# vincentjzy/OpenCorr

Measured on NVIDIA H100. Metric: POIs/sec (FFTCC+ICGN to convergence), higher is better.
Workload: dtype f32

## Files before the change

opencorr_b200/csrc/fft32.cuh:

```cuda
#pragma once
#include "ocb_common.cuh"

namespace ocb {

__host__ __device__ constexpr int brev5(int i) {
	return ((i & 1) << 4) | ((i & 2) << 2) | (i & 4) | ((i & 8) >> 2) | ((i & 16) >> 4);
}

__device__ __forceinline__ float tw32_cos(int k) {
	switch (k) {
	case 0: return 1.0f;
	case 1: return 0.98078528040323044913f;
	case 2: return 0.92387953251128675613f;
	case 3: return 0.83146961230254523708f;
	case 4: return 0.70710678118654752440f;
	case 5: return 0.55557023301960222474f;
	case 6: return 0.38268343236508977173f;
	case 7: return 0.19509032201612826785f;
	case 8: return 0.0f;
	case 9: return -0.19509032201612826785f;
	case 10: return -0.38268343236508977173f;
	case 11: return -0.55557023301960222474f;
	case 12: return -0.70710678118654752440f;
	case 13: return -0.83146961230254523708f;
	case 14: return -0.92387953251128675613f;
	default: return -0.98078528040323044913f;
	}
}
__device__ __forceinline__ float tw32_sin(int k) { return k < 8 ? tw32_cos(8 - k) : tw32_cos(k - 8); }

template <bool INV>
__device__ __forceinline__ void mul_tw32(float xr, float xi, int k, float& yr, float& yi) {
	if (k == 0) {
		yr = xr;
		yi = xi;
	} else if (k == 8) {
		yr = INV ? -xi : xi;
		yi = INV ? xr : -xr;
	} else {
		const float c = tw32_cos(k), s = INV ? -tw32_sin(k) : tw32_sin(k);
		yr = fmaf(xr, c, xi * s);
		yi = fmaf(xi, c, -xr * s);
	}
}

template <bool INV, int HALF>
__device__ __forceinline__ void fft32_dif_stage(float* re, float* im) {
#pragma unroll
	for (int base = 0; base < 32; base += 2 * HALF) {
#pragma unroll
		for (int k = 0; k < HALF; k++) {
			const int i = base + k, j = i + HALF;
			const float ar = re[i], ai = im[i], br = re[j], bi = im[j];
			re[i] = ar + br;
			im[i] = ai + bi;
			mul_tw32<INV>(ar - br, ai - bi, k * (16 / HALF), re[j], im[j]);
		}
	}
}

template <bool INV, int HALF>
__device__ __forceinline__ void fft32_dit_stage(float* re, float* im) {
#pragma unroll
	for (int base = 0; base < 32; base += 2 * HALF) {
#pragma unroll
		for (int k = 0; k < HALF; k++) {
			const int i = base + k, j = i + HALF;
			float tr, ti;
			mul_tw32<INV>(re[j], im[j], k * (16 / HALF), tr, ti);
			const float ar = re[i], ai = im[i];
			re[i] = ar + tr;
			im[i] = ai + ti;
			re[j] = ar - tr;
			im[j] = ai - ti;
		}
	}
}

template <bool INV>
__device__ __forceinline__ void fft32_dif(float* re, float* im) {
	fft32_dif_stage<INV, 16>(re, im);
	fft32_dif_stage<INV, 8>(re, im);
	fft32_dif_stage<INV, 4>(re, im);
	fft32_dif_stage<INV, 2>(re, im);
	fft32_dif_stage<INV, 1>(re, im);
}

template <bool INV>
__device__ __forceinline__ void fft32_dit(float* re, float* im) {
	fft32_dit_stage<INV, 1>(re, im);
	fft32_dit_stage<INV, 2>(re, im);
	fft32_dit_stage<INV, 4>(re, im);
	fft32_dit_stage<INV, 8>(re, im);
	fft32_dit_stage<INV, 16>(re, im);
}

}
```

opencorr_b200/csrc/fftcc2d_w32.cu:

```cuda
#include <stdlib.h>
#include <string.h>

#include "fft32.cuh"
#include "fftcc_common.cuh"
#include "ocb_kernels.h"
#include "ocb_tma.cuh"

namespace ocb {

constexpr int FFTW32_PITCH = 33;
constexpr int FFTW32_BOX_W = 36;
constexpr int FFTW32_TILE = 32 * FFTW32_BOX_W;

__global__ void __launch_bounds__(FFTW32_WARPS * 32) fftcc2d_w32_kernel(Image2D img, float* __restrict__ pois, int n_poi,
	const __grid_constant__ CUtensorMap tm_ref, const __grid_constant__ CUtensorMap tm_tar, int use_tma) {
	__shared__ __align__(128) float s_re[FFTW32_WARPS][FFTW32_TILE];
	__shared__ __align__(128) float s_im[FFTW32_WARPS][FFTW32_TILE];
	__shared__ __align__(8) uint64_t s_bar[FFTW32_WARPS];
	constexpr int R = 16, M = 32 * 32;
	const int lane = threadIdx.x & 31, warp = threadIdx.x >> 5;
	float* sre = s_re[warp];
	float* sim = s_im[warp];
	uint64_t* bar = &s_bar[warp];
	uint32_t bar_phase = 0;
	if (use_tma) {
		if (lane == 0) mbar_init(bar, 1);
		__syncwarp();
	}
	const int w = img.w, h = img.h;
	const int plane = (32 - lane) & 31;

	const int poi_stride = gridDim.x * FFTW32_WARPS;
	int poi = blockIdx.x * FFTW32_WARPS + warp;
	float rec_next = (poi < n_poi && lane < P2_N) ? pois[(size_t)poi * P2_N + lane] : 0.f;
	for (; poi < n_poi; poi += poi_stride) {
		float* P = pois + (size_t)poi * P2_N;
		const float rec = rec_next;
		if (poi + poi_stride < n_poi && lane < P2_N) rec_next = pois[(size_t)(poi + poi_stride) * P2_N + lane];
		const float px = __shfl_sync(0xffffffffu, rec, P2_X), py = __shfl_sync(0xffffffffu, rec, P2_Y);
		const float u0 = __shfl_sync(0xffffffffu, rec, P2_DEF + D2_U), v0 = __shfl_sync(0xffffffffu, rec, P2_DEF + D2_V);
		if (fftcc2d_skip(px, py, u0, v0, R, R, w, h)) continue;
		float re[32], im[32];
		{
			float sa = 0.f, sb = 0.f;
			if (use_tma && px == floorf(px) && py == floorf(py) && u0 == floorf(u0) && v0 == floorf(v0)) {
				const int x0r = (int)px - R, y0r = (int)py - R, x0t = (int)(px + u0) - R, y0t = (int)(py + v0) - R;
				const int axr = floor4(x0r), axt = floor4(x0t);
				if (lane == 0) {
					fence_proxy_async();
					mbar_expect_tx(bar, (uint32_t)(2 * FFTW32_TILE * sizeof(float)));
					tma_load_2d(sre, &tm_ref, axr, y0r, bar);
					tma_load_2d(sim, &tm_tar, axt, y0t, bar);
				}
				mbar_wait(bar, bar_phase);
				bar_phase ^= 1;
				const float* cr = sre + (x0r - axr) + lane;
				const float* ci = sim + (x0t - axt) + lane;
#pragma unroll
				for (int r = 0; r < 32; r++) {
					re[r] = cr[r * FFTW32_BOX_W];
					im[r] = ci[r * FFTW32_BOX_W];
					sa += re[r];
					sb += im[r];
				}
			} else {
				const float rpx = px + lane - R;
				const int ax = (int)rpx, bx = (int)(rpx + u0);
#pragma unroll
				for (int r = 0; r < 32; r++) {
					const float rpy = py + r - R;
					re[r] = __ldg(img.ref + (size_t)(int)rpy * w + ax);
					im[r] = __ldg(img.tar + (size_t)(int)(rpy + v0) * w + bx);
					sa += re[r];
					sb += im[r];
				}
			}
			sa = warp_sum(sa) / (float)M;
			sb = warp_sum(sb) / (float)M;
#pragma unroll
			for (int r = 0; r < 32; r++) {
				re[r] -= sa;
				im[r] -= sb;
			}
		}
		float na = 0.f, nb = 0.f;
#pragma unroll
		for (int r = 0; r < 32; r++) {
			na = fmaf(re[r], re[r], na);
			nb = fmaf(im[r], im[r], nb);
		}
		na = warp_sum(na);
		nb = warp_sum(nb);

		fft32_dif<false>(re, im);
		__syncwarp();
#pragma unroll
		for (int i = 0; i < 32; i++) {
			sre[brev5(i) * FFTW32_PITCH + lane] = re[i];
			sim[brev5(i) * FFTW32_PITCH + lane] = im[i];
		}
		__syncwarp();
#pragma unroll
		for (int i = 0; i < 32; i++) {
			re[i] = sre[lane * FFTW32_PITCH + i];
			im[i] = sim[lane * FFTW32_PITCH + i];
		}
		fft32_dif<false>(re, im);

#pragma unroll
		for (int i = 0; i < 32; i++) {
			const int ip = brev5((32 - brev5(i)) & 31);
			if (ip < i) continue;
			const float pr_i = __shfl_sync(0xffffffffu, re[i], plane), pi_i = __shfl_sync(0xffffffffu, im[i], plane);
			if (ip == i) {
				cross_spectrum(re[i], im[i], pr_i, pi_i);
			} else {
				const float pr_p = __shfl_sync(0xffffffffu, re[ip], plane), pi_p = __shfl_sync(0xffffffffu, im[ip], plane);
				cross_spectrum(re[i], im[i], pr_p, pi_p);
				cross_spectrum(re[ip], im[ip], pr_i, pi_i);
			}
		}

		fft32_dit<true>(re, im);
		__syncwarp();
#pragma unroll
		for (int i = 0; i < 32; i++) {
			sre[lane * FFTW32_PITCH + i] = re[i];
			sim[lane * FFTW32_PITCH + i] = im[i];
		}
		__syncwarp();
#pragma unroll
		for (int i = 0; i < 32; i++) {
			re[i] = sre[brev5(i) * FFTW32_PITCH + lane];
			im[i] = sim[brev5(i) * FFTW32_PITCH + lane];
		}
		fft32_dit<true>(re, im);

		float bv = -2.f;
		int bi = 0;
#pragma unroll
		for (int y = 0; y < 32; y++) {
			if (re[y] > bv) { bv = re[y]; bi = y * 32 + lane; }
		}
		warp_argmax(bv, bi);
		{
			const Fftcc2dResult res = fftcc2d_result(bv, bi, na, nb, R, R, u0, v0);
			float out = 0.f;
			if (lane == P2_DEF + D2_U) out = res.u;
			if (lane == P2_DEF + D2_V) out = res.v;
			if (lane == P2_U0) out = u0;
			if (lane == P2_V0) out = v0;
			if (lane == P2_ZNCC) out = res.zncc;
			if (lane == P2_DEF + D2_U || lane == P2_DEF + D2_V || lane == P2_U0 || lane == P2_V0 || lane == P2_ZNCC) P[lane] = out;
		}
		__syncwarp();
	}
}

int fftcc2d_w32_launch(const Image2D& img, float* d_pois, size_t n, int grid, cudaStream_t stream, cudaError_t* err) {
	CUtensorMap tm_ref, tm_tar;
	memset(&tm_ref, 0, sizeof(tm_ref));
	memset(&tm_tar, 0, sizeof(tm_tar));
	const int dims[2] = { img.w, img.h }, box[2] = { FFTW32_BOX_W, 32 };
	const int use_tma = !getenv("OCB_NO_TMA") && tma_make_map(&tm_ref, img.ref, 2, dims, box) && tma_make_map(&tm_tar, img.tar, 2, dims, box);
	fftcc2d_w32_kernel<<<grid, FFTW32_WARPS * 32, 0, stream>>>(img, d_pois, (int)n, tm_ref, tm_tar, use_tma);
	*err = cudaGetLastError();
	return *err == cudaSuccess ? 0 : -2;
}

}
```

opencorr_b200/csrc/fftcc_common.cuh:

```cuda
#pragma once
#include "ocb_common.cuh"

namespace ocb {

__device__ __forceinline__ bool fftcc2d_skip(float px, float py, float u0, float v0, int rx, int ry, int w, int h) {
	return (int)px < rx || (int)px >= w - rx || (int)py < ry || (int)py >= h - ry || (int)(px + u0) < rx || (int)(px + u0) >= w - rx
		|| (int)(py + v0) < ry || (int)(py + v0) >= h - ry || is_nan_f(px) || is_nan_f(py) || is_nan_f(u0) || is_nan_f(v0);
}

__device__ __forceinline__ bool fftcc3d_skip(float px, float py, float pz, float u0, float v0, float w0, int rx, int ry, int rz, int dx, int dy,
	int dz) {
	const int sx = 2 * rx, sy = 2 * ry, sz = 2 * rz;
	const int x0 = (int)(px - rx), y0 = (int)(py - ry), z0 = (int)(pz - rz);
	const int x1 = (int)(px + (sx - 1) - rx), y1 = (int)(py + (sy - 1) - ry), z1 = (int)(pz + (sz - 1) - rz);
	const int tx0 = (int)(px - rx + u0), ty0 = (int)(py - ry + v0), tz0 = (int)(pz - rz + w0);
	const int tx1 = (int)(px + (sx - 1) - rx + u0), ty1 = (int)(py + (sy - 1) - ry + v0), tz1 = (int)(pz + (sz - 1) - rz + w0);
	return x0 < 0 || y0 < 0 || z0 < 0 || x1 >= dx || y1 >= dy || z1 >= dz || tx0 < 0 || ty0 < 0 || tz0 < 0 || tx1 >= dx || ty1 >= dy || tz1 >= dz
		|| px - rx < 0 || py - ry < 0 || pz - rz < 0 || px - rx + u0 < 0 || py - ry + v0 < 0 || pz - rz + w0 < 0
		|| is_nan_f(px) || is_nan_f(py) || is_nan_f(pz) || is_nan_f(u0) || is_nan_f(v0) || is_nan_f(w0);
}

__device__ __forceinline__ void cross_spectrum(float& re, float& im, float nr, float ni) {
	const float Ar = 0.5f * (re + nr), Ai = 0.5f * (im - ni);
	const float dr = 0.5f * (re - nr), di = 0.5f * (im + ni);
	const float Br = di, Bi = -dr;
	re = Ar * Br + Ai * Bi;
	im = Ar * Bi - Ai * Br;
}

__device__ __forceinline__ void argmax_merge(float& bv, int& bi, float v, int i) {
	if (v > bv || (v == bv && i < bi)) { bv = v; bi = i; }
}
__device__ __forceinline__ void warp_argmax(float& bv, int& bi) {
#pragma unroll
	for (int o = 16; o > 0; o >>= 1) {
		const float ov = __shfl_xor_sync(0xffffffffu, bv, o);
		const int oi = __shfl_xor_sync(0xffffffffu, bi, o);
		argmax_merge(bv, bi, ov, oi);
	}
}

__device__ __forceinline__ void fftcc_constant_window(float& bv, int& bi, float na, float nb) {
	if (na == 0.f || nb == 0.f) { bv = 0.f; bi = 0; }
}
__device__ __forceinline__ float fftcc_zncc(float bv, float na, float nb, int m) { return bv / (sqrtf(na * nb) * (float)m); }
__device__ __forceinline__ int fftcc_wrap(int d, int r) { return d > r ? d - 2 * r : d; }

struct Fftcc2dResult {
	float u, v, zncc;
};
__device__ __forceinline__ Fftcc2dResult fftcc2d_result(float bv, int bi, float na, float nb, int rx, int ry, float u0, float v0) {
	fftcc_constant_window(bv, bi, na, nb);
	const int sw = 2 * rx;
	const unsigned k = (unsigned)bi;
	return { (float)fftcc_wrap((int)(k % sw), rx) + u0, (float)fftcc_wrap((int)(k / sw), ry) + v0, fftcc_zncc(bv, na, nb, sw * 2 * ry) };
}
__device__ __forceinline__ void fftcc2d_store(float* P, float bv, int bi, float na, float nb, int rx, int ry, float u0, float v0) {
	const Fftcc2dResult r = fftcc2d_result(bv, bi, na, nb, rx, ry, u0, v0);
	P[P2_DEF + D2_U] = r.u;
	P[P2_DEF + D2_V] = r.v;
	P[P2_U0] = u0;
	P[P2_V0] = v0;
	P[P2_ZNCC] = r.zncc;
}

__device__ __forceinline__ void fftcc3d_store(float* P, float bv, int bi, float na, float nb, int rx, int ry, int rz, float u0, float v0, float w0) {
	fftcc_constant_window(bv, bi, na, nb);
	const int sx = 2 * rx, sy = 2 * ry;
	const unsigned k = (unsigned)bi;
	P[P3_DEF + 0] = (float)fftcc_wrap((int)(k % sx), rx) + u0;
	P[P3_DEF + 4] = (float)fftcc_wrap((int)(k / sx % sy), ry) + v0;
	P[P3_DEF + 8] = (float)fftcc_wrap((int)(k / (sx * sy)), rz) + w0;
	P[P3_U0] = u0;
	P[P3_V0] = v0;
	P[P3_W0] = w0;
	P[P3_ZNCC] = fftcc_zncc(bv, na, nb, sx * sy * 2 * rz);
}

}
```

Measured before the change: 50.44 million.

## Exploit real-valued correlation output with half-size inverse FFT and float2 transposes

Replaces the full 32x32 complex inverse FFT with a real-output split: one 32-point pass becomes a twiddle pre-step plus a 16-point FFT. The second pass is handled by splitting lanes into two halves that each do a 16-point FFT over half the rows. The transpose buffers are merged into one float2 shared tile so each element moves with one vector access. The cross-spectrum drops its 0.5 scaling, and the factor is restored once at the argmax. This trims FFT arithmetic and shared-memory traffic, but the index mapping and argmax tie-breaking logic become more intricate.

```diff
diff --git a/opencorr_b200/csrc/fft32.cuh b/opencorr_b200/csrc/fft32.cuh
--- a/opencorr_b200/csrc/fft32.cuh
+++ b/opencorr_b200/csrc/fft32.cuh
@@ -44,10 +44,10 @@
 	}
 }
 
-template <bool INV, int HALF>
-__device__ __forceinline__ void fft32_dif_stage(float* re, float* im) {
+template <int N, bool INV, int HALF>
+__device__ __forceinline__ void fft_dif_stage(float* re, float* im) {
 #pragma unroll
-	for (int base = 0; base < 32; base += 2 * HALF) {
+	for (int base = 0; base < N; base += 2 * HALF) {
 #pragma unroll
 		for (int k = 0; k < HALF; k++) {
 			const int i = base + k, j = i + HALF;
@@ -59,10 +59,10 @@
 	}
 }
 
-template <bool INV, int HALF>
-__device__ __forceinline__ void fft32_dit_stage(float* re, float* im) {
+template <int N, bool INV, int HALF>
+__device__ __forceinline__ void fft_dit_stage(float* re, float* im) {
 #pragma unroll
-	for (int base = 0; base < 32; base += 2 * HALF) {
+	for (int base = 0; base < N; base += 2 * HALF) {
 #pragma unroll
 		for (int k = 0; k < HALF; k++) {
 			const int i = base + k, j = i + HALF;
@@ -79,20 +79,56 @@
 
 template <bool INV>
 __device__ __forceinline__ void fft32_dif(float* re, float* im) {
-	fft32_dif_stage<INV, 16>(re, im);
-	fft32_dif_stage<INV, 8>(re, im);
-	fft32_dif_stage<INV, 4>(re, im);
-	fft32_dif_stage<INV, 2>(re, im);
-	fft32_dif_stage<INV, 1>(re, im);
+	fft_dif_stage<32, INV, 16>(re, im);
+	fft_dif_stage<32, INV, 8>(re, im);
+	fft_dif_stage<32, INV, 4>(re, im);
+	fft_dif_stage<32, INV, 2>(re, im);
+	fft_dif_stage<32, INV, 1>(re, im);
 }
 
 template <bool INV>
 __device__ __forceinline__ void fft32_dit(float* re, float* im) {
-	fft32_dit_stage<INV, 1>(re, im);
-	fft32_dit_stage<INV, 2>(re, im);
-	fft32_dit_stage<INV, 4>(re, im);
-	fft32_dit_stage<INV, 8>(re, im);
-	fft32_dit_stage<INV, 16>(re, im);
+	fft_dit_stage<32, INV, 1>(re, im);
+	fft_dit_stage<32, INV, 2>(re, im);
+	fft_dit_stage<32, INV, 4>(re, im);
+	fft_dit_stage<32, INV, 8>(re, im);
+	fft_dit_stage<32, INV, 16>(re, im);
+}
+
+template <bool INV>
+__device__ __forceinline__ void fft16_dif(float* re, float* im) {
+	fft_dif_stage<16, INV, 8>(re, im);
+	fft_dif_stage<16, INV, 4>(re, im);
+	fft_dif_stage<16, INV, 2>(re, im);
+	fft_dif_stage<16, INV, 1>(re, im);
+}
+
+template <bool INV>
+__device__ __forceinline__ void fft16_dit(float* re, float* im) {
+	fft_dit_stage<16, INV, 1>(re, im);
+	fft_dit_stage<16, INV, 2>(re, im);
+	fft_dit_stage<16, INV, 4>(re, im);
+	fft_dit_stage<16, INV, 8>(re, im);
+}
+
+__device__ __forceinline__ void ifft32_real_split(float* re, float* im) {
+#pragma unroll
+	for (int j = 0; j < 16; j++) {
+		const int k = brev5(2 * j);
+		const float ar = re[2 * j], ai = im[2 * j], br = re[2 * j + 1], bi = im[2 * j + 1];
+		if (k == 0) {
+			re[j] = (ar + br) - (ai - bi);
+			im[j] = (ai + bi) + (ar - br);
+		} else if (k == 8) {
+			re[j] = br + br;
+			im[j] = bi + bi;
+		} else {
+			const float er = ar + br, ei = ai + bi, dr = ar - br, di = ai - bi;
+			const float c = tw32_cos(k), s = tw32_sin(k);
+			re[j] = fmaf(-dr, s, fmaf(-di, c, er));
+			im[j] = fmaf(dr, c, fmaf(-di, s, ei));
+		}
+	}
 }
 
 }
diff --git a/opencorr_b200/csrc/fftcc2d_w32.cu b/opencorr_b200/csrc/fftcc2d_w32.cu
--- a/opencorr_b200/csrc/fftcc2d_w32.cu
+++ b/opencorr_b200/csrc/fftcc2d_w32.cu
@@ -11,16 +11,17 @@
 constexpr int FFTW32_PITCH = 33;
 constexpr int FFTW32_BOX_W = 36;
 constexpr int FFTW32_TILE = 32 * FFTW32_BOX_W;
+static_assert(32 * FFTW32_PITCH * 2 <= 2 * FFTW32_TILE, "the transpose tile must fit in the two boxes");
 
 __global__ void __launch_bounds__(FFTW32_WARPS * 32) fftcc2d_w32_kernel(Image2D img, float* __restrict__ pois, int n_poi,
 	const __grid_constant__ CUtensorMap tm_ref, const __grid_constant__ CUtensorMap tm_tar, int use_tma) {
-	__shared__ __align__(128) float s_re[FFTW32_WARPS][FFTW32_TILE];
-	__shared__ __align__(128) float s_im[FFTW32_WARPS][FFTW32_TILE];
+	__shared__ __align__(128) float s_buf[FFTW32_WARPS][2 * FFTW32_TILE];
 	__shared__ __align__(8) uint64_t s_bar[FFTW32_WARPS];
 	constexpr int R = 16, M = 32 * 32;
 	const int lane = threadIdx.x & 31, warp = threadIdx.x >> 5;
-	float* sre = s_re[warp];
-	float* sim = s_im[warp];
+	float* sre = s_buf[warp];
+	float* sim = s_buf[warp] + FFTW32_TILE;
+	float2* st = reinterpret_cast<float2*>(s_buf[warp]);
 	uint64_t* bar = &s_bar[warp];
 	uint32_t bar_phase = 0;
 	if (use_tma) {
@@ -95,15 +96,13 @@
 		fft32_dif<false>(re, im);
 		__syncwarp();
 #pragma unroll
-		for (int i = 0; i < 32; i++) {
-			sre[brev5(i) * FFTW32_PITCH + lane] = re[i];
-			sim[brev5(i) * FFTW32_PITCH + lane] = im[i];
-		}
+		for (int i = 0; i < 32; i++) st[brev5(i) * FFTW32_PITCH + lane] = make_float2(re[i], im[i]);
 		__syncwarp();
 #pragma unroll
 		for (int i = 0; i < 32; i++) {
-			re[i] = sre[lane * FFTW32_PITCH + i];
-			im[i] = sim[lane * FFTW32_PITCH + i];
+			const float2 v = st[lane * FFTW32_PITCH + i];
+			re[i] = v.x;
+			im[i] = v.y;
 		}
 		fft32_dif<false>(re, im);
 
@@ -113,38 +112,50 @@
 			if (ip < i) continue;
 			const float pr_i = __shfl_sync(0xffffffffu, re[i], plane), pi_i = __shfl_sync(0xffffffffu, im[i], plane);
 			if (ip == i) {
-				cross_spectrum(re[i], im[i], pr_i, pi_i);
+				cross_spectrum4(re[i], im[i], pr_i, pi_i);
 			} else {
 				const float pr_p = __shfl_sync(0xffffffffu, re[ip], plane), pi_p = __shfl_sync(0xffffffffu, im[ip], plane);
-				cross_spectrum(re[i], im[i], pr_p, pi_p);
-				cross_spectrum(re[ip], im[ip], pr_i, pi_i);
+				cross_spectrum4(re[i], im[i], pr_p, pi_p);
+				cross_spectrum4(re[ip], im[ip], pr_i, pi_i);
 			}
 		}
 
-		fft32_dit<true>(re, im);
+		ifft32_real_split(re, im);
+		fft16_dit<true>(re, im);
 		__syncwarp();
 #pragma unroll
-		for (int i = 0; i < 32; i++) {
-			sre[lane * FFTW32_PITCH + i] = re[i];
-			sim[lane * FFTW32_PITCH + i] = im[i];
+		for (int n = 0; n < 16; n++) st[lane * FFTW32_PITCH + n] = make_float2(re[n], im[n]);
+		__syncwarp();
+		const int n = lane & 15, h = lane >> 4;
+		const float hf = (float)h, sgn = 1.f - 2.f * hf;
+#pragma unroll
+		for (int ky = 0; ky < 16; ky++) {
+			const float2 a = st[ky * FFTW32_PITCH + n], b = st[(ky + 16) * FFTW32_PITCH + n];
+			const float tr = fmaf(sgn, b.x, a.x), ti = fmaf(sgn, b.y, a.y);
+			if (ky == 0) {
+				re[ky] = tr;
+				im[ky] = ti;
+			} else {
+				const float cm1 = tw32_cos(ky) - 1.f, s = tw32_sin(ky);
+				re[ky] = fmaf(hf, fmaf(tr, cm1, -ti * s), tr);
+				im[ky] = fmaf(hf, fmaf(ti, cm1, tr * s), ti);
+			}
 		}
-		__syncwarp();
+		fft16_dif<true>(re, im);
+
+		float bv = -8.f;
+		const int i0 = h * 32 + 2 * n;
+		int bi = -i0;
 #pragma unroll
-		for (int i = 0; i < 32; i++) {
-			re[i] = sre[brev5(i) * FFTW32_PITCH + lane];
-			im[i] = sim[brev5(i) * FFTW32_PITCH + lane];
+		for (int m = 0; m < 16; m++) {
+			const int j = brev5(2 * m);
+			if (re[j] > bv) { bv = re[j]; bi = m * 64; }
+			if (im[j] > bv) { bv = im[j]; bi = m * 64 + 1; }
 		}
-		fft32_dit<true>(re, im);
-
-		float bv = -2.f;
-		int bi = 0;
-#pragma unroll
-		for (int y = 0; y < 32; y++) {
-			if (re[y] > bv) { bv = re[y]; bi = y * 32 + lane; }
-		}
+		bi += i0;
 		warp_argmax(bv, bi);
 		{
-			const Fftcc2dResult res = fftcc2d_result(bv, bi, na, nb, R, R, u0, v0);
+			const Fftcc2dResult res = fftcc2d_result(0.25f * bv, bi, na, nb, R, R, u0, v0);
 			float out = 0.f;
 			if (lane == P2_DEF + D2_U) out = res.u;
 			if (lane == P2_DEF + D2_V) out = res.v;
diff --git a/opencorr_b200/csrc/fftcc_common.cuh b/opencorr_b200/csrc/fftcc_common.cuh
--- a/opencorr_b200/csrc/fftcc_common.cuh
+++ b/opencorr_b200/csrc/fftcc_common.cuh
@@ -23,6 +23,13 @@
 __device__ __forceinline__ void cross_spectrum(float& re, float& im, float nr, float ni) {
 	const float Ar = 0.5f * (re + nr), Ai = 0.5f * (im - ni);
 	const float dr = 0.5f * (re - nr), di = 0.5f * (im + ni);
+	const float Br = di, Bi = -dr;
+	re = Ar * Br + Ai * Bi;
+	im = Ar * Bi - Ai * Br;
+}
+__device__ __forceinline__ void cross_spectrum4(float& re, float& im, float nr, float ni) {
+	const float Ar = re + nr, Ai = im - ni;
+	const float dr = re - nr, di = im + ni;
 	const float Br = di, Bi = -dr;
 	re = Ar * Br + Ai * Bi;
 	im = Ar * Bi - Ai * Br;
```

Measured after the change: 52.06 million (median of 6 runs). 1.03x the previous value.
